# thelondonsmiths/Solex_ser_recon_EN

Measured on AMD Instinct MI355X. Metric: SER frames/sec end-to-end (decode→clahe) + %HBM roofline, 1/2/4/8 MI355X, higher is better.
Workload: dtype u16

## Files before the change

### include/shg_hip.h

```cpp
#ifndef SHG_HIP_H
#define SHG_HIP_H

#include <stddef.h>
#include <stdint.h>

#ifdef __cplusplus
extern "C" {
#endif

#define SHG_ABI_VERSION 16

#define SHG_E_ARG        (-1)
#define SHG_E_WORKSPACE  (-2)
#define SHG_E_UNSUPPORTED (-3)
#define SHG_E_VALUE      (-4)
#define SHG_E_TYPE       (-5)
#define SHG_E_LINALG     (-6)
#define SHG_E_RUNTIME    (-7)
#define SHG_E_QHULL      (-8)
#define SHG_E_ASSERT     (-9)
#define SHG_E_INDEX      (-10)

typedef void* shg_stream_t;

// ... 145 lines not shown
                        int64_t n_cols, int64_t k_offset, int flip_x, shg_stream_t stream);

int shg_extract_columns_minmax(const void* stack, int64_t n_frames, int64_t height, int64_t width,
                               int bytes_per_px, int64_t frame_stride_px, const int32_t* ind_l, const double* lw, const double* rw,
                               int n_shifts, uint16_t* disks, int64_t row_pitch, int64_t plane_stride,
                               int64_t n_cols, int64_t k_offset, int flip_x, uint32_t* minmax_slots, shg_stream_t stream);

int shg_extract_dense_fits(const int32_t* host_shifts, int n_shifts);
int shg_extract_columns_dense(const void* stack, int64_t n_frames, int64_t height, int64_t width, int bytes_per_px,
                              int64_t frame_stride_px, const int32_t* ind_l, const int32_t* base_col, const double* lw,
                              const double* rw, const int32_t* host_shifts, int n_shifts, uint16_t* disks, int64_t row_pitch,
                              int64_t plane_stride, int64_t n_cols, int64_t k_offset, int flip_x, uint32_t* minmax_slots,
                              shg_stream_t stream);

int shg_warp_rows_u16(const uint16_t* src, int64_t h, int64_t w, int64_t src_pitch,
                      double h00, double h01, double h02,
                      uint16_t* dst, int64_t out_h, int64_t out_w, int64_t dst_pitch,
                      uint32_t* minmax, shg_stream_t stream);

int shg_warp_rows_minmax_u16(const uint16_t* src, int64_t h, int64_t w, int64_t src_pitch,
                             double h00, double h01, double h02,
                             uint16_t* dst, int64_t out_h, int64_t out_w, int64_t dst_pitch,
                             const uint32_t* minmax2, shg_stream_t stream);

int shg_warp_rows_wide_fits(const uint16_t* src, int64_t h, int64_t w, int64_t src_pitch,
                            double h00, double h01, double h02,
                            const uint16_t* dst, int64_t out_h, int64_t out_w, int64_t dst_pitch);

#define SHG_TRANSV_MAX_COLS 19456
int shg_rowpair_logratio_stats(const uint16_t* img, int64_t h, int64_t w, int64_t pitch,
                               int64_t y1, int64_t y2, const int32_t* xa, const int32_t* xb,
                               const double* row_factor, double* out, shg_stream_t stream);
int shg_rowpair_logratio_stats_mirrored(const uint16_t* img, int64_t h, int64_t w, int64_t pitch,
                                        int64_t y1, int64_t y2, const int32_t* xa, const int32_t* xb,
                                        const double* row_factor, double* out, double* out_mirror, shg_stream_t stream);

int shg_correlate1d_rows_f64(const double* src, int64_t k, int64_t n, const double* weights, int radius,
                             int symmetric, double* dst, shg_stream_t stream);

int shg_scale_rows_u16(const uint16_t* img, int64_t h, int64_t w, int64_t pitch, const double* c,
                       const double* row_factor, uint16_t* dst, int64_t dst_pitch, shg_stream_t stream);
int shg_scale_rows_vec_fits(const uint16_t* img, int64_t h, int64_t w, int64_t pitch, const uint16_t* dst, int64_t dst_pitch);

int shg_lin_filter_row_sums(const uint16_t* img, int64_t h, int64_t w, int64_t pitch,
                            const double* row_factor, const float* log_lut, const uint8_t* flagged,
                            const int32_t* up, const int32_t* dn, int linlen, double* hl, double* hf,
// ... 269 lines not shown
```

### solex_ser_recon_en_amd/_lib.py

```python
import ctypes
import os
from ctypes import c_double, c_int, c_int32, c_int64, c_size_t, c_uint16, c_uint32, c_void_p

import torch

_HERE = os.path.dirname(os.path.abspath(__file__))
LIB_PATH = os.path.join(_HERE, 'csrc', 'libshg_hip.so')

if not os.path.exists(LIB_PATH):
    raise ImportError(
        'libshg_hip.so is missing (%s). Build it with `python -c "import __graft_entry__ as g; g.build()"` or '
        '`make -C solex_ser_recon_en_amd/csrc`. There is no CPU fallback for the SHG hot path.' % LIB_PATH)

lib = ctypes.CDLL(LIB_PATH)

P = c_void_p
PD = ctypes.POINTER(c_double)
PI64 = ctypes.POINTER(c_int64)


class ScanRequest(ctypes.Structure):
    _fields_ = [('struct_bytes', c_uint32), ('start_phase', c_int32),
                ('stack', P), ('n_frames', c_int64), ('height', c_int64), ('width', c_int64), ('frame_stride_px', c_int64),
                ('bytes_per_px', c_int32), ('flip_x', c_int32),
# ... 73 lines not shown
    'shg_patch_ssd_u16': (c_int, [P, c_int64, P, c_int64, c_int64, c_int64, P, c_int64, c_int, c_int, P, P, P]),
    'shg_stack_combine_field_u16': (c_int, [P, P, P, P, c_int64, c_int64, c_int, c_int, c_int, c_double, c_int, P, c_int64, c_int64, c_int64,
                                            P, c_int64, P]),
    'shg_patch_sharpness_u16': (c_int, [P, c_int64, c_int64, c_int64, P, c_int64, c_int, c_int, P, P, P]),
    'shg_stack_combine_weighted_u16': (c_int, [P, P, P, P, P, c_int64, c_int64, c_int, c_int, c_int, c_double, c_int, P, c_int64, c_int64,
                                               c_int64, P, c_int64, P]),
    'shg_wavelet_workspace_bytes': (c_size_t, [c_int64, c_int64, c_int]),
    'shg_wavelet_sharpen_u16': (c_int, [P, c_int64, c_int64, c_int64, c_int, P, P, P, c_int64, P, P, c_size_t, P]),
    'shg_wavelet_noise_u16': (c_int, [P, c_int64, c_int64, c_int64, P, P, P, c_size_t, P]),
    'shg_rl_workspace_bytes': (c_size_t, [c_int64, c_int64]),
    'shg_rl_deconvolve_u16': (c_int, [P, c_int64, c_int64, c_int64, P, c_int, c_int, P, c_int64, P, P, c_size_t, P]),
    'shg_blur_fits_fused': (c_int, [c_int64, c_int]),
    'shg_blur_row_mean_u16': (c_int, [P, c_int64, c_int64, c_int, c_int, P, P]),
    'shg_blur_argmin_u16': (c_int, [P, c_int64, c_int64, c_int, c_int, c_int64, c_int64, P, P, P]),
    'shg_extract_columns': (c_int, [P, c_int64, c_int64, c_int64, c_int, c_int64, P, P, P, c_int, P, c_int64, c_int64,
                                    c_int64, c_int64, c_int, P]),
    'shg_extract_columns_minmax': (c_int, [P, c_int64, c_int64, c_int64, c_int, c_int64, P, P, P, c_int, P, c_int64, c_int64,
                                           c_int64, c_int64, c_int, P, P]),
    'shg_extract_dense_fits': (c_int, [P, c_int]),
    'shg_extract_columns_dense': (c_int, [P, c_int64, c_int64, c_int64, c_int, c_int64, P, P, P, P, P, c_int, P, c_int64, c_int64, c_int64, c_int64,
                                          c_int, P, P]),
    'shg_warp_rows_minmax_u16': (c_int, [P, c_int64, c_int64, c_int64, c_double, c_double, c_double, P, c_int64, c_int64,
                                         c_int64, P, P]),
    'shg_warp_rows_u16': (c_int, [P, c_int64, c_int64, c_int64, c_double, c_double, c_double, P, c_int64, c_int64,
                                  c_int64, P, P]),
    'shg_warp_rows_wide_fits': (c_int, [P, c_int64, c_int64, c_int64, c_double, c_double, c_double, P, c_int64, c_int64, c_int64]),
    'shg_rowpair_logratio_stats': (c_int, [P, c_int64, c_int64, c_int64, c_int64, c_int64, P, P, P, P, P]),
    'shg_rowpair_logratio_stats_mirrored': (c_int, [P, c_int64, c_int64, c_int64, c_int64, c_int64, P, P, P, P, P, P]),
    'shg_line_order_stats_u16': (c_int, [P, c_int64, c_int64, c_int64, c_int, c_int64, c_int64, P, P, P]),
    'shg_scale_rows_u16': (c_int, [P, c_int64, c_int64, c_int64, P, P, P, c_int64, P]),
    'shg_scale_rows_vec_fits': (c_int, [P, c_int64, c_int64, c_int64, P, c_int64]),
    'shg_correlate1d_rows_f64': (c_int, [P, c_int64, c_int64, P, c_int, c_int, P, P]),
    'shg_lin_filter_row_sums': (c_int, [P, c_int64, c_int64, c_int64, P, P, P, P, P, c_int, P, P, P]),
    'shg_lin_filter_apply': (c_int, [P, c_int64, c_int64, c_int64, P, P, P, c_int, c_int, P, P, P, P, c_int, P, c_int64, P]),
    'shg_crop_pad_u16': (c_int, [P, c_int64, c_int64, c_int64, P, c_int64, c_int64, c_int64, c_int64, c_int64,
                                 c_int, P]),
    'shg_clahe_workspace_bytes': (c_size_t, [c_int, c_int]),
    'shg_clahe_workspace_bytes_for': (c_size_t, [c_int64, c_int64, c_int, c_int]),
    'shg_clahe': (c_int, [P, c_int64, c_int64, c_int64, c_int, c_double, c_int, P, c_int64, P, c_size_t, P]),
    'shg_hist': (c_int, [P, c_int64, c_int64, c_int64, c_int, P, P]),
    'shg_select_u16_workspace_bytes': (c_size_t, [c_int]),
    'shg_select_u16': (c_int, [P, c_int64, c_int64, c_int64, ctypes.POINTER(c_int64), c_int, P, P, c_size_t, P]),
    'shg_rescale_u16': (c_int, [P, c_int64, c_int64, c_int64, c_double, c_double, c_double, P, c_int64, P]),
    'shg_rescale_u8': (c_int, [P, c_int64, c_int64, c_int64, c_double, c_double, c_double, P, c_int64, P]),
    'shg_contrast_stats_workspace_bytes': (c_size_t, [c_int]),
    'shg_contrast_stats_workspace_bytes_for': (c_size_t, [c_int64, c_int64, c_int]),
# ... 224 lines not shown
```

### solex_ser_recon_en_amd/csrc/scan.hip

```cpp
#include <math.h>
#include <string.h>
#include <atomic>
#include <vector>
#include "shg_common.h"

namespace {

constexpr size_t kAlign = 256;
inline size_t up(size_t b) { return (b + kAlign - 1) / kAlign * kAlign; }
inline int64_t round64(int64_t v) { return (v + 63) / 64 * 64; }
inline int64_t floor_div(int64_t a, int64_t b) { int64_t q = a / b; return (a % b != 0 && ((a < 0) != (b < 0))) ? q - 1 : q; }

const double kRadToDeg = 180.0 / 3.141592653589793238462643383279502884;
const double kDegToRad = 3.141592653589793238462643383279502884 / 180.0;

std::atomic<shg_savgol_taps_fn> g_taps_fn{nullptr};

#define SCAN_TRY(expr)                  \
    do {                                \
        if (int e_ = (expr)) return e_; \
    } while (0)

struct Regions {
    size_t mean_ws, extract_ws, limb_ws, mean_pin, extract_pin, limb_pin, process_pin;
// ... 268 lines not shown
    std::vector<double> w_h;
    auto add_warp = [&](int i, uint16_t* dst) {
        const double* hr = i == 0 ? rs->h_first : rs->h_rest;
        w_src.push_back(rq->disks + (size_t)i * rq->disk_plane_stride);
        w_dst.push_back(dst);
        w_mm.push_back(extrema + 2 * i);
        w_h.insert(w_h.end(), hr, hr + 3);
    };
    if (fit_image) add_warp(0, reinterpret_cast<uint16_t*>(arena + rs->fit_image_off));
    std::vector<const uint16_t*> frames((size_t)k);
    std::vector<uint16_t*> det((size_t)k), prod[5];
    for (auto& v : prod) v.resize((size_t)k);
    int64_t j = 0;
    for (int i = 0; i < S; ++i) {
        if (!rq->host_requested[i]) continue;
        uint16_t* f = reinterpret_cast<uint16_t*>(arena + rs->frames_off + (size_t)j * frame_bytes);
        add_warp(i, f);
        frames[j] = f;
        if (detrans) det[j] = reinterpret_cast<uint16_t*>(arena + rs->detrans_off + (size_t)j * frame_bytes);
        for (int p = 0; p < 3; ++p) prod[p][j] = reinterpret_cast<uint16_t*>(arena + rs->products_off + ((size_t)j * 3 + p) * prod_bytes);
        for (int p = 0; p < 2; ++p) prod[3 + p][j] = reinterpret_cast<uint16_t*>(results + ((size_t)j * 2 + p) * prod_bytes);
        ++j;
    }
    if (!w_src.empty())
        SCAN_TRY(shg::warp_rows_batch(w_src.data(), (int64_t)w_src.size(), ih, n_cols, rq->disk_pitch, w_h.data(), w_dst.data(), out_h, out_w, frame_pitch,
                                      w_mm.data(), stream));
    if (k > 0) {
        SCAN_TRY(shg_stage_process_frames(frames.data(), k, out_h, out_w, frame_pitch, rq->transversalium, pl.trans_circle, pl.trans_borders,
                                          pl.taps_ptr, pl.window, rq->host_factors, pl.crop_w, pl.sx0, pl.dx0, pl.ncopy, rq->clip_limit, rq->tiles,
                                          pl.disc[0], pl.disc[1], pl.disc[2], detrans ? det.data() : nullptr, frame_pitch, prod[0].data(),
                                          prod[1].data(), prod[2].data(), prod[3].data(), prod[4].data(), prod_pitch, process_ws, process_ws_bytes,
                                          process_pin, rg.process_pin, stream));
    }
    rs->phase_done = 4;
    return 0;
}
```

### solex_ser_recon_en_amd/csrc/shg_common.h

```cpp
#pragma once
#if defined(__HIPCC__)
#include <hip/hip_runtime.h>
#include <hip/hip_ext.h>
#endif
#include <stdint.h>
#include <stdio.h>
#include <string.h>
#include <type_traits>

#if defined(__HIPCC__)
#define SHG_HD __host__ __device__ __forceinline__
#else
#define SHG_HD inline
#endif

namespace shg {

SHG_HD uint64_t f64_key(double v) {
#if defined(__HIP_DEVICE_COMPILE__)
    const uint64_t b = (uint64_t)__double_as_longlong(v);
#else
    uint64_t b;
    memcpy(&b, &v, sizeof b);
#endif
// ... 111 lines not shown
    template <typename T>
    __device__ __forceinline__ T* at(int i) const { return static_cast<T*>(const_cast<void*>(p[i])); }
};
using PtrBatch = PtrBatchN<kMaxBatch>;
template <int N, typename T>
inline PtrBatchN<N> make_batch_n(T* const* host_ptrs, int first, int count) {
    PtrBatchN<N> b = {};
    for (int i = 0; i < count && i < N; ++i) b.p[i] = host_ptrs[first + i];
    return b;
}
template <typename T>
inline PtrBatch make_batch(T* const* host_ptrs, int first, int count) { return make_batch_n<kMaxBatch>(host_ptrs, first, count); }

int rowpair_stats_batch(const uint16_t* const* host_imgs, int64_t k, int64_t h, int64_t w, int64_t pitch, int64_t y1, int64_t y2,
                        const int32_t* xa, const int32_t* xb, const double* row_factor, double* out, double* out_mirror, shg_stream_t stream);
int scale_rows_batch(const uint16_t* const* host_imgs, int64_t k, int64_t h, int64_t w, int64_t pitch, const double* c,
                     const double* row_factor, uint16_t* const* host_dsts, int64_t dst_pitch, shg_stream_t stream);
int crop_pad_batch(const uint16_t* const* host_srcs, int64_t k, int64_t h, int64_t w, int64_t pitch, uint16_t* const* host_dsts, int64_t nw,
                   int64_t dst_pitch, int64_t sx0, int64_t dx0, int64_t n, int32_t fill, shg_stream_t stream);
int contrast_products_batch(const uint16_t* const* host_frames, int64_t frame_pitch, const uint16_t* const* host_cl1, int64_t cl1_pitch,
                            int64_t k, int64_t h, int64_t w, const double* host_lo_hi6, uint16_t* const* host_hc, uint16_t* const* host_protus,
                            uint16_t* const* host_cc, int64_t dst_pitch, int64_t disc_x0, int64_t disc_y0, int64_t disc_r, shg_stream_t stream,
                            const double* stats5 = nullptr, double g_bright = 0.0, double g_dark = 0.0, double* mirror5 = nullptr);
int warp_rows_batch(const uint16_t* const* host_srcs, int64_t k, int64_t h, int64_t w, int64_t src_pitch, const double* host_h3,
                    uint16_t* const* host_dsts, int64_t out_h, int64_t out_w, int64_t dst_pitch, const uint32_t* const* host_minmax2,
                    shg_stream_t stream);
struct FrameSource {
    const uint16_t* const* host_raw;
    int64_t raw_pitch;
    const double* factors;
    int64_t sx0, dx0, ncopy;
};
bool contrast_stats_batches(int64_t h, int64_t w, int tiles, double clip_limit);
int contrast_stats_batch(const uint16_t* const* host_frames, int64_t k, int64_t h, int64_t w, int64_t pitch, double clip_limit, int tiles,
                         uint16_t* const* host_cl1, int64_t cl1_pitch, const int64_t* ranks_frame2, const int64_t* ranks_cl13, double* out5,
                         void* workspace, size_t workspace_bytes, shg_stream_t stream, const FrameSource* from = nullptr);

constexpr int kWave = 64;
constexpr int kCUs = 256;

__device__ __forceinline__ int lane_id() { return threadIdx.x & (kWave - 1); }

template <typename Op>
__device__ __forceinline__ uint32_t wave_fold_u32(uint32_t v, Op op) {
    v = op(v, (uint32_t)__builtin_amdgcn_update_dpp((int)v, (int)v, 0xB1, 0xf, 0xf, false));
    v = op(v, (uint32_t)__builtin_amdgcn_update_dpp((int)v, (int)v, 0x4E, 0xf, 0xf, false));
    v = op(v, (uint32_t)__builtin_amdgcn_update_dpp((int)v, (int)v, 0x141, 0xf, 0xf, false));
    v = op(v, (uint32_t)__builtin_amdgcn_update_dpp((int)v, (int)v, 0x140, 0xf, 0xf, false));
    const uint32_t r0 = (uint32_t)__builtin_amdgcn_readlane((int)v, 0), r1 = (uint32_t)__builtin_amdgcn_readlane((int)v, 16),
// ... 89 lines not shown
```

### solex_ser_recon_en_amd/csrc/stages.hip

```cpp
#include <math.h>
#include <stdlib.h>
#include <string.h>
#include <algorithm>
#include <vector>
#include "shg_common.h"

namespace {

constexpr size_t kAlign = 256;
inline size_t up(size_t b) { return (b + kAlign - 1) / kAlign * kAlign; }

struct Arena {
    char* base;
    size_t cap, off;
    Arena(void* p, size_t bytes) : base(static_cast<char*>(p)), cap(bytes), off(0) {}
    template <typename T>
    T* take(size_t count) {
        const size_t b = up(count * sizeof(T));
        if (!base || off + b > cap) return nullptr;
        T* p = reinterpret_cast<T*>(base + off);
        off += b;
        return p;
    }
};
// ... 49 lines not shown
    if (n_words == 0) return 0;
    const unsigned blocks = (unsigned)std::min<size_t>((n_words + 255) / 256, 64);
    return shg::launch(k_words, dim3(blocks), dim3(256), 0, st, WordsArgs{static_cast<uint32_t*>(dst), static_cast<const uint32_t*>(src), n_words, nullptr, 0}, "k_words");
}

struct Staging {
    char* host;
    char* dev;
    template <typename T>
    T* on_device(T* host_ptr) const { return reinterpret_cast<T*>(dev + (reinterpret_cast<char*>(host_ptr) - host)); }
};

inline int map_staging(void* host_pinned, Staging* out, const char* who) {
    void* d = nullptr;
    hipError_t e = hipHostGetDevicePointer(&d, host_pinned, 0);
    if (e != hipSuccess || !d) {
        (void)hipGetLastError();
        shg::set_error("%s: host_pinned is not page-locked, GPU-mapped memory (hipHostMalloc / hipHostRegister): %s", who,
                       e != hipSuccess ? hipGetErrorString(e) : "no device address");
        return SHG_E_ARG;
    }
    out->host = static_cast<char*>(host_pinned);
    out->dev = static_cast<char*>(d);
    return 0;
}

inline int64_t slit_rows(int64_t height, int64_t width) { return width > height ? width : height; }
inline int64_t spectral_cols(int64_t height, int64_t width) { return width > height ? height : width; }

}

extern "C" size_t shg_stage_mean_fit_workspace_bytes(int64_t n_frames, int64_t height, int64_t width, int bytes_per_px) {
    if (height <= 0 || width <= 0) return 0;
    const size_t hw = (size_t)height * (size_t)width, ih = (size_t)slit_rows(height, width);
    const size_t acc = n_frames > 0 ? shg_accumulate_workspace_bytes(n_frames, height, width, bytes_per_px) : 0;
    return up(acc) + up(hw * 8) + up(hw * 2) + up(hw * 2) + up(hw * 4) + up(ih * 8) + up(2 * ih * 4) + kAlign;
}

extern "C" size_t shg_stage_mean_fit_host_bytes(int64_t height, int64_t width) {
    if (height <= 0 || width <= 0) return 0;
    const size_t ih = (size_t)slit_rows(height, width);
    return up(ih * 8) + up(2 * ih * 4);
}

extern "C" int shg_stage_mean_fit(const void* stack, int64_t n_frames, int64_t height, int64_t width, int bytes_per_px,
                                  int64_t frame_stride_px, const uint64_t* sum_in, const uint16_t* max_in, int64_t n_total,
// ... 331 lines not shown
        if (host_flags[i]) {
            X[2 * j] = (double)host_points[2 * i] * kFactor;
            X[2 * j + 1] = (double)host_points[2 * i + 1] * kFactor;
            ++j;
        }
    STAGE_TRY(shg_host_limb_geometry(X.data(), n_sel, h, w, host_geom16, host_dims2, kept.data(), &host_counts3[2], host_outline200));
    for (int64_t i = 0, j = 0; i < m; ++i)
        if (host_flags[i]) { if (kept[j]) host_flags[i] |= 2; ++j; }
    return 0;
}

extern "C" size_t shg_stage_process_workspace_bytes(int64_t k, int64_t h, int64_t w, int64_t crop_w, int tiles) {
    if (k <= 0 || h <= 0 || w <= 0) return 0;
    const size_t pitch = ((size_t)std::max(w, crop_w) + 63) / 64 * 64;
    return 2 * up((size_t)h * 4) + 2 * up((size_t)k * h * 8) + up((size_t)k * h * 8) + up(4096 * 8) +
           (size_t)k * up((size_t)h * pitch * 2) + (size_t)k * up(shg_contrast_stats_workspace_bytes_for(h, crop_w > 0 ? crop_w : w, tiles)) + up((size_t)k * 5 * 8) + kAlign;
}

extern "C" size_t shg_stage_process_host_bytes(int64_t k, int64_t h) {
    if (k <= 0 || h <= 0) return 0;
    return 2 * up((size_t)h * 4) + 2 * up((size_t)k * h * 8) + up((size_t)k * h * 8) + up((size_t)k * 5 * 8) + up(4096 * 8);
}

extern "C" int shg_stage_process_frames(const uint16_t* const* host_frames, int64_t k, int64_t h, int64_t w, int64_t pitch,
                                        int transversalium, const double* host_circle3, const double* host_borders4,
                                        const double* host_taps, int64_t window, double* host_factors,
                                        int64_t crop_w, int64_t sx0, int64_t dx0, int64_t ncopy,
                                        double clip_limit, int tiles, int64_t disc_x0, int64_t disc_y0, int64_t disc_r,
                                        uint16_t* const* host_detrans, int64_t detrans_pitch,
                                        uint16_t* const* host_final, uint16_t* const* host_cl1, uint16_t* const* host_hc,
                                        uint16_t* const* host_protus, uint16_t* const* host_cc, int64_t out_pitch,
                                        void* workspace, size_t workspace_bytes, void* host_pinned, size_t host_pinned_bytes,
                                        shg_stream_t stream) {
    SHG_HOST_TIME("stage process_frames");
    SHG_REQUIRE(host_frames && host_final && host_cl1 && host_hc && host_protus && host_cc && workspace && host_pinned, SHG_E_ARG,
                "shg_stage_process_frames: null pointer");
    SHG_REQUIRE(k > 0 && h > 0 && w > 0 && pitch >= w, SHG_E_ARG, "shg_stage_process_frames: bad image size");
    const int64_t out_w = crop_w > 0 ? crop_w : w;
    SHG_REQUIRE(out_pitch >= out_w, SHG_E_ARG, "shg_stage_process_frames: out_pitch < output width");
    hipStream_t st = shg::as_stream(stream);
    Arena dev(workspace, workspace_bytes), pin(host_pinned, host_pinned_bytes);
    int32_t* xa = dev.take<int32_t>((size_t)h);
    int32_t* xb = dev.take<int32_t>((size_t)h);
    double* taps_d = dev.take<double>(4096);
    double* stats = dev.take<double>((size_t)k * h);
    double* interior = dev.take<double>((size_t)k * h);
    double* factors = dev.take<double>((size_t)k * h);
    const size_t tpitch = ((size_t)w + 63) / 64 * 64;
    std::vector<uint16_t*> scaled((size_t)k, nullptr);
    const char* fuse_env = getenv("SHG_FUSE_SCALE");
    const bool fuse_on = !(fuse_env && fuse_env[0] == '0');
    const bool fuse = fuse_on && !host_detrans && shg::contrast_stats_batches(h, crop_w > 0 ? crop_w : w, tiles, clip_limit) && pitch >= w;
    const bool need_tmp = transversalium && crop_w > 0 && !host_detrans && !fuse;
    if (need_tmp)
        for (int64_t i = 0; i < k; ++i) scaled[i] = dev.take<uint16_t>((size_t)h * tpitch);
    const size_t cs_each = up(shg_contrast_stats_workspace_bytes_for(h, out_w, tiles));
    SHG_REQUIRE(cs_each != 0, SHG_E_ARG, "shg_stage_process_frames: unsupported tile count %d", tiles);
    const size_t cs_bytes = (size_t)k * cs_each;
    char* cs_ws = dev.take<char>(cs_bytes);
    double* out5 = dev.take<double>((size_t)k * 5);
    int32_t* h_xa = pin.take<int32_t>((size_t)h);
    int32_t* h_xb = pin.take<int32_t>((size_t)h);
    double* h_taps = pin.take<double>(4096);
    double* h_stats = pin.take<double>((size_t)k * h);
    double* h_interior = pin.take<double>((size_t)k * h);
    double* h_factors = pin.take<double>((size_t)k * h);
    double* h_out5 = pin.take<double>((size_t)k * 5);
    SHG_REQUIRE(xa && xb && stats && interior && factors && taps_d && cs_ws && out5 && (!need_tmp || scaled[k - 1]), SHG_E_WORKSPACE,
                "shg_stage_process_frames: workspace too small");
    SHG_REQUIRE(h_xa && h_xb && h_stats && h_interior && h_factors && h_out5 && h_taps, SHG_E_WORKSPACE, "shg_stage_process_frames: pinned staging area too small");
    Staging stg;
    STAGE_TRY(map_staging(host_pinned, &stg, "shg_stage_process_frames"));

    std::vector<const uint16_t*> cur((size_t)k);
    int64_t cur_pitch = pitch;
    for (int64_t i = 0; i < k; ++i) cur[i] = host_frames[i];
    if (transversalium) {
        SHG_REQUIRE(host_circle3 && host_borders4 && host_taps, SHG_E_ARG, "shg_stage_process_frames: transversalium needs circle, borders, taps");
        const double cx = host_circle3[0], cy = host_circle3[1], r = host_circle3[2];
        const int64_t y1 = (int64_t)ceil(std::max(cy - r, host_borders4[1])), y2 = (int64_t)floor(std::min(cy + r, host_borders4[3]));
        int64_t n = 1;
        bool have_rows = y2 - y1 >= 1;
        const double* use_interior = nullptr;
        if (have_rows) {
            SHG_REQUIRE(y1 >= 0 && y2 <= h, SHG_E_ARG, "shg_stage_process_frames: rows [%lld, %lld) outside the image", (long long)y1, (long long)y2);
            n = y2 - y1;
            STAGE_TRY(shg_host_chord_bounds(cx, cy, r, host_borders4[0], host_borders4[2], y1, y2, w, h_xa, h_xb));
            const bool gpu_interior = window > 3 && window <= n && window / 2 <= 1024 && window <= 4096;
            std::vector<double> rev;
            if (gpu_interior) {
                rev.resize((size_t)window);
                for (int64_t i = 0; i < window; ++i) rev[i] = host_taps[window - 1 - i];
                memcpy(h_taps, rev.data(), (size_t)window * 8);
            }
            const char* plan_end = gpu_interior ? reinterpret_cast<const char*>(h_taps + window) : reinterpret_cast<const char*>(h_xb + n);
            STAGE_TRY(move_words(xa, stg.on_device(h_xa), (size_t)(plan_end - reinterpret_cast<const char*>(h_xa)), st));
            STAGE_TRY(shg::rowpair_stats_batch(host_frames, k, h, w, pitch, y1, y2, xa, xb, nullptr, stats, stg.on_device(h_stats), stream));
            if (gpu_interior) {
                const int radius = (int)(window / 2);
                int sym = 1, anti = 1;
                for (int i = 1; i <= radius; ++i) {
                    if (fabs(rev[radius + i] - rev[radius - i]) > 2.220446049250313e-16) sym = 0;
                    if (fabs(rev[radius + i] + rev[radius - i]) > 2.220446049250313e-16) anti = 0;
                }
                STAGE_TRY(shg_correlate1d_rows_f64(stats, k, n, taps_d, radius, sym ? 1 : (anti ? -1 : 0), stg.on_device(h_interior), stream));
                use_interior = h_interior;
            }
            STAGE_SYNC(st, "shg_stage_process_frames");
        } else {
            for (int64_t i = 0; i < k; ++i) h_stats[i] = 0.0;
        }
        std::vector<double> corr((size_t)k * n);
        STAGE_TRY(shg_host_transversalium_factors(h_stats, use_interior, k, n, host_taps, window, 1, corr.data()));
        for (int64_t i = 0; i < k; ++i) {
            double* c = h_factors + i * h;
            for (int64_t y = 0; y < h; ++y) c[y] = 1.0;
            if (have_rows) memcpy(c + y1, corr.data() + i * n, (size_t)n * 8);
        }
        if (host_factors) memcpy(host_factors, h_factors, (size_t)k * h * 8);
        factors = stg.on_device(h_factors);
      if (!fuse) {
        std::vector<uint16_t*> dsts((size_t)k);
        int64_t dpitch = out_pitch;
        for (int64_t i = 0; i < k; ++i) {
            if (host_detrans) { dsts[i] = host_detrans[i]; dpitch = detrans_pitch; }
            else if (crop_w > 0) { dsts[i] = scaled[i]; dpitch = (int64_t)tpitch; }
            else { dsts[i] = host_final[i]; dpitch = out_pitch; }
            SHG_REQUIRE(dsts[i] && dpitch >= w, SHG_E_ARG, "shg_stage_process_frames: bad de-transversalium output");
// ... 49 lines not shown
```

### solex_ser_recon_en_amd/csrc/warp.hip

```cpp
#include <algorithm>
#include <cmath>
#include "shg_common.h"
#include <type_traits>

namespace {

__global__ void k_minmax_init(uint32_t* mm) {
    mm[0] = 0xffffffffu;
    mm[1] = 0u;
}

__global__ __launch_bounds__(256) void k_minmax(const uint16_t* __restrict__ src, int64_t h, int64_t w, int64_t pitch,
                                                uint32_t* __restrict__ mm) {
    uint32_t lo = 0xffffffffu, hi = 0u;
    for (int64_t y0 = blockIdx.x; y0 < h; y0 += 8 * (int64_t)gridDim.x) {
        for (int64_t x = threadIdx.x; x < w; x += 256) {
            uint32_t v[8];
            bool ok[8];
#pragma unroll
            for (int u = 0; u < 8; ++u) {
                const int64_t y = y0 + u * (int64_t)gridDim.x;
                ok[u] = y < h;
                v[u] = src[(ok[u] ? y : y0) * pitch + x];
            }
// ... 14 lines not shown
    }
    __shared__ uint32_t wlo[4], whi[4];
    if ((threadIdx.x & 63) == 0) { wlo[threadIdx.x >> 6] = lo; whi[threadIdx.x >> 6] = hi; }
    __syncthreads();
    if (threadIdx.x == 0) {
        for (int i = 1; i < 4; ++i) { lo = wlo[i] < lo ? wlo[i] : lo; hi = whi[i] > hi ? whi[i] : hi; }
        atomicMin(&mm[0], lo);
        atomicMax(&mm[1], hi);
    }
}

constexpr int kWarpBatch = 24;
struct WarpRows { double h[kWarpBatch][3]; };

using WarpPtrs = shg::PtrBatchN<kWarpBatch>;
struct WarpArgs {
    WarpPtrs srcs;
    int64_t h, w, pitch;
    WarpRows rows;
    WarpPtrs dsts;
    int64_t out_h, out_w, dst_pitch;
    WarpPtrs mms;
    uint32_t nv_magic, nv_shift;
};

template <int WARP_ROWS>
__global__ __launch_bounds__(256) void k_warp_rows(const WarpArgs kargs) {
    const WarpPtrs& srcs = kargs.srcs;
    const WarpPtrs& dsts = kargs.dsts;
    const WarpPtrs& mms = kargs.mms;
    const int64_t h = kargs.h, w = kargs.w, pitch = kargs.pitch, out_h = kargs.out_h, out_w = kargs.out_w, dst_pitch = kargs.dst_pitch;
    const WarpRows& rows = kargs.rows;
    const uint16_t* __restrict__ src = srcs.at<const uint16_t>(blockIdx.z);
    uint16_t* __restrict__ dst = dsts.at<uint16_t>(blockIdx.z);
    const uint32_t* __restrict__ mm = mms.at<const uint32_t>(blockIdx.z);
    const double h00 = rows.h[blockIdx.z][0], h01 = rows.h[blockIdx.z][1], h02 = rows.h[blockIdx.z][2];
    const int c = (int)(blockIdx.x * 256 + threadIdx.x);
    const int ra = (int)blockIdx.y * WARP_ROWS;
    if (c >= out_w) return;
    double dc[WARP_ROWS];
    uint32_t v0[WARP_ROWS], v1[WARP_ROWS];
    bool in0[WARP_ROWS], in1[WARP_ROWS];
    const bool sane = fabs(h00) < 1e300 && fabs(h01) < 1e300 && fabs(h02) < 1e300;
    const uint32_t wu = (uint32_t)w;
    const double xc = h00 * (double)c;
#pragma unroll
    for (int rr = 0; rr < WARP_ROWS; ++rr) {
        const int r = ra + rr;
        const double x = xc + h01 * (double)r + h02;
        const double x0 = floor(x);
// ... 6 lines not shown
        const uint16_t* row = src + (int64_t)(row_ok ? r : 0) * pitch;
        v0[rr] = row[in0[rr] ? i0 : 0];
        v1[rr] = row[in1[rr] ? i1 : 0];
    }
    const uint32_t cval = src[0];
    const double lo = (double)mm[0], hi = (double)mm[1];
#pragma unroll
    for (int rr = 0; rr < WARP_ROWS; ++rr) {
        const int r = ra + rr;
        if (r >= out_h) break;
        const double left = (double)(in0[rr] ? v0[rr] : cval), right = (double)(in1[rr] ? v1[rr] : cval);
        double v = (1.0 - dc[rr]) * left + dc[rr] * right;
        v = fmin(fmax(v, lo), hi);
        dst[(int64_t)r * dst_pitch + c] = (uint16_t)(int)v;
    }
}

typedef unsigned int __attribute__((ext_vector_type(4))) u32x4_t;
typedef unsigned int __attribute__((ext_vector_type(3))) u32x3_t;
constexpr int kWarpPairs = 22;
template <int ITER>
__global__ __launch_bounds__(256) __attribute__((amdgpu_waves_per_eu(7))) void k_warp_rows8(const WarpArgs kargs) {
    __shared__ uint32_t win[4][kWarpPairs][64];
    const int64_t h = kargs.h, w = kargs.w, pitch = kargs.pitch, out_h = kargs.out_h, out_w = kargs.out_w, dst_pitch = kargs.dst_pitch;
    const uint16_t* __restrict__ src = kargs.srcs.at<const uint16_t>(blockIdx.z);
    uint16_t* __restrict__ dst = kargs.dsts.at<uint16_t>(blockIdx.z);
    const uint32_t* __restrict__ mm = kargs.mms.at<const uint32_t>(blockIdx.z);
    const double h00 = kargs.rows.h[blockIdx.z][0], h01 = kargs.rows.h[blockIdx.z][1], h02 = kargs.rows.h[blockIdx.z][2];
    const uint32_t nv = (uint32_t)((out_w + 7) / 8), total = nv * (uint32_t)out_h;
    const int lane = threadIdx.x & 63, wave = threadIdx.x >> 6;
    uint32_t (*const my)[64] = win[wave];
    const uint32_t cval = src[0];
    const int lo_i = (int)mm[0], hi_i = (int)mm[1];
    const double k00 = h00 * 0x1p+52;
    const uint32_t wu = (uint32_t)w;
    const int w_last = (int)w - 1, last_piece = (int)pitch - 8;

    auto place = [&](int it, int& r, int& c, int& ws, double& hr, double& x) {
        const uint32_t flat = ((uint32_t)blockIdx.x * ITER + (uint32_t)it) * 256u + threadIdx.x;
        const uint32_t f = flat < total ? flat : total - 1;
        r = (int)(__umulhi(f, kargs.nv_magic) >> kargs.nv_shift);
        c = (int)(f - (uint32_t)r * nv) * 8;
        hr = h01 * (double)r;
        x = h00 * (double)c + hr + h02;
        const int i0 = __double2int_rz(floor(x));
        ws = min(max(i0, 0), w_last) & ~7;
// ... 100 lines not shown
                                 uint32_t* minmax, shg_stream_t stream) {
    SHG_REQUIRE(src && dst && minmax, SHG_E_ARG, "shg_warp_rows_u16: null pointer");
    SHG_REQUIRE(h > 0 && w > 0 && out_h > 0 && out_w > 0, SHG_E_ARG, "shg_warp_rows_u16: empty image");
    SHG_REQUIRE(src_pitch >= w && dst_pitch >= out_w, SHG_E_ARG, "shg_warp_rows_u16: pitch smaller than width");
    SHG_REQUIRE(out_h < 65536, SHG_E_UNSUPPORTED, "shg_warp_rows_u16: more than 65535 rows");
    hipStream_t st = shg::as_stream(stream);
    { SHG_PROF("minmax", st); k_minmax_init<<<1, 1, 0, st>>>(minmax); }
    int64_t blocks = h < 256 ? h : 256;
    { SHG_PROF("minmax", st); k_minmax<<<(unsigned)blocks, 256, 0, st>>>(src, h, w, src_pitch, minmax); }
    if (int e = shg::check_launch("k_minmax")) return e;
    const double h3[3] = {h00, h01, h02};
    const uint32_t* mm = minmax;
    return shg::warp_rows_batch(&src, 1, h, w, src_pitch, h3, &dst, out_h, out_w, dst_pitch, &mm, stream);
}

extern "C" int shg_warp_rows_minmax_u16(const uint16_t* src, int64_t h, int64_t w, int64_t src_pitch, double h00, double h01,
                                        double h02, uint16_t* dst, int64_t out_h, int64_t out_w, int64_t dst_pitch,
                                        const uint32_t* minmax2, shg_stream_t stream) {
    SHG_REQUIRE(src && dst && minmax2, SHG_E_ARG, "shg_warp_rows_minmax_u16: null pointer");
    const double h3[3] = {h00, h01, h02};
    return shg::warp_rows_batch(&src, 1, h, w, src_pitch, h3, &dst, out_h, out_w, dst_pitch, &minmax2, stream);
}

int shg::warp_rows_batch(const uint16_t* const* host_srcs, int64_t k, int64_t h, int64_t w, int64_t src_pitch, const double* host_h3,
                         uint16_t* const* host_dsts, int64_t out_h, int64_t out_w, int64_t dst_pitch, const uint32_t* const* host_minmax2,
                         shg_stream_t stream) {
    SHG_REQUIRE(host_srcs && host_h3 && host_dsts && host_minmax2 && k > 0, SHG_E_ARG, "shg_warp_rows_minmax_u16: null pointer");
    SHG_REQUIRE(h > 0 && w > 0 && out_h > 0 && out_w > 0, SHG_E_ARG, "shg_warp_rows_minmax_u16: empty image");
    SHG_REQUIRE(src_pitch >= w && dst_pitch >= out_w, SHG_E_ARG, "shg_warp_rows_minmax_u16: pitch smaller than width");
    SHG_REQUIRE(out_h < 65536 && out_w < (1ll << 30) && w < (1ll << 30) && h < (1ll << 30), SHG_E_UNSUPPORTED, "shg_warp_rows_minmax_u16: image too large");
    for (int64_t i = 0; i < k; ++i) SHG_REQUIRE(host_srcs[i] && host_dsts[i] && host_minmax2[i], SHG_E_ARG, "shg_warp_rows_minmax_u16: null image");
    hipStream_t st = shg::as_stream(stream);
    SHG_PROF("warp", st);
    for (int64_t i0 = 0; i0 < k; i0 += kWarpBatch) {
        const int m = (int)std::min<int64_t>(kWarpBatch, k - i0);
        WarpRows rows = {};
        for (int d = 0; d < m; ++d)
            for (int j = 0; j < 3; ++j) rows.h[d][j] = host_h3[3 * (i0 + d) + j];
        const uint64_t nv = (uint64_t)((out_w + 7) / 8);
        uint32_t nv_shift = 0;
        while ((2ull << nv_shift) < nv) ++nv_shift;
        const uint32_t nv_magic = nv >= 2 ? (uint32_t)(((1ull << (32 + nv_shift)) + nv - 1) / nv) : 0u;
        const WarpArgs args{shg::make_batch_n<kWarpBatch>(host_srcs, (int)i0, m), h, w, src_pitch, rows, shg::make_batch_n<kWarpBatch>(host_dsts, (int)i0, m),
                            out_h, out_w, dst_pitch, shg::make_batch_n<kWarpBatch>(host_minmax2, (int)i0, m), nv_magic, nv_shift};
        const bool wide_ok = [] { const char* e = getenv("SHG_WARP_WIDE"); return !e || atoi(e) != 0; }();
        bool wide = wide_ok;
        for (int d = 0; d < m && wide; ++d)
            wide = shg_warp_rows_wide_fits(host_srcs[i0 + d], h, w, src_pitch, rows.h[d][0], rows.h[d][1], rows.h[d][2], host_dsts[i0 + d], out_h, out_w, dst_pitch) != 0;
        if (wide) {
            const int64_t vecs = out_h * ((out_w + 7) / 8);
            const bool few = vecs * m < 4 * 256 * 2048;
            auto go8 = [&](auto I) {
                dim3 grid((unsigned)((vecs + 256 * I.value - 1) / (256 * I.value)), 1u, (unsigned)m);
                return shg::launch(k_warp_rows8<I.value>, grid, dim3(256), 0, st, args, "k_warp_rows8");
            };
            if (int e = few ? go8(std::integral_constant<int, 1>{}) : go8(std::integral_constant<int, 4>{})) return e;
            continue;
        }
        const int64_t gx = (out_w + 255) / 256;
        int rows_per_lane = gx * ((out_h + 7) / 8) * m >= kWarpWideAbove ? 8 : 4;
        if (warp_rows_forced()) rows_per_lane = warp_rows_forced();
        auto go = [&](auto R) {
            dim3 grid((unsigned)gx, (unsigned)((out_h + R.value - 1) / R.value), (unsigned)m);
            return shg::launch(k_warp_rows<R.value>, grid, dim3(256), 0, st, args, "k_warp_rows");
        };
        const int e = rows_per_lane == 16 ? go(std::integral_constant<int, 16>{})
                    : rows_per_lane == 8 ? go(std::integral_constant<int, 8>{}) : go(std::integral_constant<int, 4>{});
// ... 5 lines not shown
```

Measured before the change: 6.099 million.

## Carry transversalium plan upload inside warp kernel to skip separate copy

The host-side transversalium plan (chord bounds, reversed taps, symmetry) is now computed before the warp launch. The warp kernels copy the plan words from mapped pinned memory to the device workspace using their first 64 workgroups. The process stage reuses that staged plan through a thread-local pointer and skips its own move_words launch. This removes one small copy launch per call, at the cost of a hidden thread-local handoff and extra work in the first warp blocks.

Result: no change. 6.060 million (-0.6%).

```diff
diff --git a/include/shg_hip.h b/include/shg_hip.h
--- a/include/shg_hip.h
+++ b/include/shg_hip.h
@@ -191,6 +191,12 @@
                              double h00, double h01, double h02,
                              uint16_t* dst, int64_t out_h, int64_t out_w, int64_t dst_pitch,
                              const uint32_t* minmax2, shg_stream_t stream);
+
+int shg_warp_rows_side_copy_u16(const uint16_t* src, int64_t h, int64_t w, int64_t src_pitch,
+                                double h00, double h01, double h02,
+                                uint16_t* dst, int64_t out_h, int64_t out_w, int64_t dst_pitch,
+                                const uint32_t* minmax2, uint32_t* side_dst, const uint32_t* side_src, size_t n_words,
+                                shg_stream_t stream);
 
 int shg_warp_rows_wide_fits(const uint16_t* src, int64_t h, int64_t w, int64_t src_pitch,
                             double h00, double h01, double h02,
diff --git a/solex_ser_recon_en_amd/_lib.py b/solex_ser_recon_en_amd/_lib.py
--- a/solex_ser_recon_en_amd/_lib.py
+++ b/solex_ser_recon_en_amd/_lib.py
@@ -119,6 +119,8 @@
                                           c_int, P, P]),
     'shg_warp_rows_minmax_u16': (c_int, [P, c_int64, c_int64, c_int64, c_double, c_double, c_double, P, c_int64, c_int64,
                                          c_int64, P, P]),
+    'shg_warp_rows_side_copy_u16': (c_int, [P, c_int64, c_int64, c_int64, c_double, c_double, c_double, P, c_int64, c_int64,
+                                            c_int64, P, P, P, c_size_t, P]),
     'shg_warp_rows_u16': (c_int, [P, c_int64, c_int64, c_int64, c_double, c_double, c_double, P, c_int64, c_int64,
                                   c_int64, P, P]),
     'shg_warp_rows_wide_fits': (c_int, [P, c_int64, c_int64, c_int64, c_double, c_double, c_double, P, c_int64, c_int64, c_int64]),
diff --git a/solex_ser_recon_en_amd/csrc/scan.hip b/solex_ser_recon_en_amd/csrc/scan.hip
--- a/solex_ser_recon_en_amd/csrc/scan.hip
+++ b/solex_ser_recon_en_amd/csrc/scan.hip
@@ -314,10 +314,16 @@
         for (int p = 0; p < 2; ++p) prod[3 + p][j] = reinterpret_cast<uint16_t*>(results + ((size_t)j * 2 + p) * prod_bytes);
         ++j;
     }
+    shg::ProcessPlanWords plan_words;
+    const bool carry = k > 0 && rq->transversalium;
+    if (carry)
+        SCAN_TRY(shg::process_plan_words(out_h, out_w, pl.trans_circle, pl.trans_borders, pl.taps_ptr, pl.window, process_ws, process_ws_bytes, process_pin,
+                                         rg.process_pin, &plan_words));
     if (!w_src.empty())
         SCAN_TRY(shg::warp_rows_batch(w_src.data(), (int64_t)w_src.size(), ih, n_cols, rq->disk_pitch, w_h.data(), w_dst.data(), out_h, out_w, frame_pitch,
-                                      w_mm.data(), stream));
+                                      w_mm.data(), stream, carry ? &plan_words.copy : nullptr));
     if (k > 0) {
+        if (carry) shg::t_process_plan_staged = &plan_words;
         SCAN_TRY(shg_stage_process_frames(frames.data(), k, out_h, out_w, frame_pitch, rq->transversalium, pl.trans_circle, pl.trans_borders,
                                           pl.taps_ptr, pl.window, rq->host_factors, pl.crop_w, pl.sx0, pl.dx0, pl.ncopy, rq->clip_limit, rq->tiles,
                                           pl.disc[0], pl.disc[1], pl.disc[2], detrans ? det.data() : nullptr, frame_pitch, prod[0].data(),
diff --git a/solex_ser_recon_en_amd/csrc/shg_common.h b/solex_ser_recon_en_amd/csrc/shg_common.h
--- a/solex_ser_recon_en_amd/csrc/shg_common.h
+++ b/solex_ser_recon_en_amd/csrc/shg_common.h
@@ -157,9 +157,23 @@
                             int64_t k, int64_t h, int64_t w, const double* host_lo_hi6, uint16_t* const* host_hc, uint16_t* const* host_protus,
                             uint16_t* const* host_cc, int64_t dst_pitch, int64_t disc_x0, int64_t disc_y0, int64_t disc_r, shg_stream_t stream,
                             const double* stats5 = nullptr, double g_bright = 0.0, double g_dark = 0.0, double* mirror5 = nullptr);
+struct SideCopy {
+    uint32_t* dst;
+    const uint32_t* src;
+    size_t n_words;
+};
 int warp_rows_batch(const uint16_t* const* host_srcs, int64_t k, int64_t h, int64_t w, int64_t src_pitch, const double* host_h3,
                     uint16_t* const* host_dsts, int64_t out_h, int64_t out_w, int64_t dst_pitch, const uint32_t* const* host_minmax2,
-                    shg_stream_t stream);
+                    shg_stream_t stream, const SideCopy* side = nullptr);
+struct ProcessPlanWords {
+    int64_t y1, y2;
+    bool have_rows, gpu_interior;
+    int symmetry;
+    SideCopy copy;
+};
+int process_plan_words(int64_t h, int64_t w, const double* host_circle3, const double* host_borders4, const double* host_taps, int64_t window,
+                       void* workspace, size_t workspace_bytes, void* host_pinned, size_t host_pinned_bytes, ProcessPlanWords* out);
+extern thread_local const ProcessPlanWords* t_process_plan_staged;
 struct FrameSource {
     const uint16_t* const* host_raw;
     int64_t raw_pitch;
diff --git a/solex_ser_recon_en_amd/csrc/stages.hip b/solex_ser_recon_en_amd/csrc/stages.hip
--- a/solex_ser_recon_en_amd/csrc/stages.hip
+++ b/solex_ser_recon_en_amd/csrc/stages.hip
@@ -95,6 +95,35 @@
     }
     out->host = static_cast<char*>(host_pinned);
     out->dev = static_cast<char*>(d);
+    return 0;
+}
+
+int plan_words(int64_t h, int64_t w, const double* host_circle3, const double* host_borders4, const double* host_taps, int64_t window,
+               int32_t* xa, int32_t* h_xa, int32_t* h_xb, double* h_taps, const Staging& stg, shg::ProcessPlanWords* out) {
+    SHG_REQUIRE(host_circle3 && host_borders4 && host_taps, SHG_E_ARG, "shg_stage_process_frames: transversalium needs circle, borders, taps");
+    const double cx = host_circle3[0], cy = host_circle3[1], r = host_circle3[2];
+    *out = shg::ProcessPlanWords{};
+    out->y1 = (int64_t)ceil(std::max(cy - r, host_borders4[1]));
+    out->y2 = (int64_t)floor(std::min(cy + r, host_borders4[3]));
+    out->have_rows = out->y2 - out->y1 >= 1;
+    if (!out->have_rows) return 0;
+    const int64_t y1 = out->y1, y2 = out->y2, n = y2 - y1;
+    SHG_REQUIRE(y1 >= 0 && y2 <= h, SHG_E_ARG, "shg_stage_process_frames: rows [%lld, %lld) outside the image", (long long)y1, (long long)y2);
+    STAGE_TRY(shg_host_chord_bounds(cx, cy, r, host_borders4[0], host_borders4[2], y1, y2, w, h_xa, h_xb));
+    out->gpu_interior = window > 3 && window <= n && window / 2 <= 1024 && window <= 4096;
+    if (out->gpu_interior) {
+        for (int64_t i = 0; i < window; ++i) h_taps[i] = host_taps[window - 1 - i];
+        const int64_t radius = window / 2;
+        int sym = 1, anti = 1;
+        for (int64_t i = 1; i <= radius; ++i) {
+            if (fabs(h_taps[radius + i] - h_taps[radius - i]) > 2.220446049250313e-16) sym = 0;
+            if (fabs(h_taps[radius + i] + h_taps[radius - i]) > 2.220446049250313e-16) anti = 0;
+        }
+        out->symmetry = sym ? 1 : (anti ? -1 : 0);
+    }
+    const char* plan_end = out->gpu_interior ? reinterpret_cast<const char*>(h_taps + window) : reinterpret_cast<const char*>(h_xb + n);
+    const size_t bytes = (size_t)(plan_end - reinterpret_cast<const char*>(h_xa));
+    out->copy = shg::SideCopy{reinterpret_cast<uint32_t*>(xa), reinterpret_cast<const uint32_t*>(stg.on_device(h_xa)), (bytes + 3) / 4};
     return 0;
 }
 
@@ -472,6 +501,25 @@
     return 2 * up((size_t)h * 4) + 2 * up((size_t)k * h * 8) + up((size_t)k * h * 8) + up((size_t)k * 5 * 8) + up(4096 * 8);
 }
 
+thread_local const shg::ProcessPlanWords* shg::t_process_plan_staged = nullptr;
+
+int shg::process_plan_words(int64_t h, int64_t w, const double* host_circle3, const double* host_borders4, const double* host_taps, int64_t window,
+                            void* workspace, size_t workspace_bytes, void* host_pinned, size_t host_pinned_bytes, shg::ProcessPlanWords* out) {
+    SHG_REQUIRE(out && workspace && host_pinned && h > 0 && w > 0, SHG_E_ARG, "shg_stage_process_frames: null pointer");
+    *out = shg::ProcessPlanWords{};
+    Arena dev(workspace, workspace_bytes), pin(host_pinned, host_pinned_bytes);
+    int32_t* xa = dev.take<int32_t>((size_t)h);
+    int32_t* xb = dev.take<int32_t>((size_t)h);
+    double* taps_d = dev.take<double>(4096);
+    int32_t* h_xa = pin.take<int32_t>((size_t)h);
+    int32_t* h_xb = pin.take<int32_t>((size_t)h);
+    double* h_taps = pin.take<double>(4096);
+    if (!xa || !xb || !taps_d || !h_xa || !h_xb || !h_taps) return 0;
+    Staging stg;
+    STAGE_TRY(map_staging(host_pinned, &stg, "shg_stage_process_frames"));
+    return plan_words(h, w, host_circle3, host_borders4, host_taps, window, xa, h_xa, h_xb, h_taps, stg, out);
+}
+
 extern "C" int shg_stage_process_frames(const uint16_t* const* host_frames, int64_t k, int64_t h, int64_t w, int64_t pitch,
                                         int transversalium, const double* host_circle3, const double* host_borders4,
                                         const double* host_taps, int64_t window, double* host_factors,
@@ -483,6 +531,8 @@
                                         void* workspace, size_t workspace_bytes, void* host_pinned, size_t host_pinned_bytes,
                                         shg_stream_t stream) {
     SHG_HOST_TIME("stage process_frames");
+    const shg::ProcessPlanWords* staged = shg::t_process_plan_staged;
+    shg::t_process_plan_staged = nullptr;
     SHG_REQUIRE(host_frames && host_final && host_cl1 && host_hc && host_protus && host_cc && workspace && host_pinned, SHG_E_ARG,
                 "shg_stage_process_frames: null pointer");
     SHG_REQUIRE(k > 0 && h > 0 && w > 0 && pitch >= w, SHG_E_ARG, "shg_stage_process_frames: bad image size");
@@ -526,34 +576,23 @@
     int64_t cur_pitch = pitch;
     for (int64_t i = 0; i < k; ++i) cur[i] = host_frames[i];
     if (transversalium) {
-        SHG_REQUIRE(host_circle3 && host_borders4 && host_taps, SHG_E_ARG, "shg_stage_process_frames: transversalium needs circle, borders, taps");
-        const double cx = host_circle3[0], cy = host_circle3[1], r = host_circle3[2];
-        const int64_t y1 = (int64_t)ceil(std::max(cy - r, host_borders4[1])), y2 = (int64_t)floor(std::min(cy + r, host_borders4[3]));
+        shg::ProcessPlanWords own;
+        const bool carried = staged && staged->copy.n_words > 0 && staged->copy.dst == reinterpret_cast<uint32_t*>(xa) &&
+                             staged->copy.src == reinterpret_cast<const uint32_t*>(stg.on_device(h_xa));
+        if (!carried) {
+            STAGE_TRY(plan_words(h, w, host_circle3, host_borders4, host_taps, window, xa, h_xa, h_xb, h_taps, stg, &own));
+            staged = &own;
+        }
+        const int64_t y1 = staged->y1, y2 = staged->y2;
         int64_t n = 1;
-        bool have_rows = y2 - y1 >= 1;
+        const bool have_rows = staged->have_rows;
         const double* use_interior = nullptr;
         if (have_rows) {
-            SHG_REQUIRE(y1 >= 0 && y2 <= h, SHG_E_ARG, "shg_stage_process_frames: rows [%lld, %lld) outside the image", (long long)y1, (long long)y2);
             n = y2 - y1;
-            STAGE_TRY(shg_host_chord_bounds(cx, cy, r, host_borders4[0], host_borders4[2], y1, y2, w, h_xa, h_xb));
-            const bool gpu_interior = window > 3 && window <= n && window / 2 <= 1024 && window <= 4096;
-            std::vector<double> rev;
-            if (gpu_interior) {
-                rev.resize((size_t)window);
-                for (int64_t i = 0; i < window; ++i) rev[i] = host_taps[window - 1 - i];
-                memcpy(h_taps, rev.data(), (size_t)window * 8);
-            }
-            const char* plan_end = gpu_interior ? reinterpret_cast<const char*>(h_taps + window) : reinterpret_cast<const char*>(h_xb + n);
-            STAGE_TRY(move_words(xa, stg.on_device(h_xa), (size_t)(plan_end - reinterpret_cast<const char*>(h_xa)), st));
+            if (!carried) STAGE_TRY(move_words(staged->copy.dst, staged->copy.src, staged->copy.n_words * 4, st));
             STAGE_TRY(shg::rowpair_stats_batch(host_frames, k, h, w, pitch, y1, y2, xa, xb, nullptr, stats, stg.on_device(h_stats), stream));
-            if (gpu_interior) {
-                const int radius = (int)(window / 2);
-                int sym = 1, anti = 1;
-                for (int i = 1; i <= radius; ++i) {
-                    if (fabs(rev[radius + i] - rev[radius - i]) > 2.220446049250313e-16) sym = 0;
-                    if (fabs(rev[radius + i] + rev[radius - i]) > 2.220446049250313e-16) anti = 0;
-                }
-                STAGE_TRY(shg_correlate1d_rows_f64(stats, k, n, taps_d, radius, sym ? 1 : (anti ? -1 : 0), stg.on_device(h_interior), stream));
+            if (staged->gpu_interior) {
+                STAGE_TRY(shg_correlate1d_rows_f64(stats, k, n, taps_d, (int)(window / 2), staged->symmetry, stg.on_device(h_interior), stream));
                 use_interior = h_interior;
             }
             STAGE_SYNC(st, "shg_stage_process_frames");
diff --git a/solex_ser_recon_en_amd/csrc/warp.hip b/solex_ser_recon_en_amd/csrc/warp.hip
--- a/solex_ser_recon_en_amd/csrc/warp.hip
+++ b/solex_ser_recon_en_amd/csrc/warp.hip
@@ -60,10 +60,24 @@
     int64_t out_h, out_w, dst_pitch;
     WarpPtrs mms;
     uint32_t nv_magic, nv_shift;
+    uint32_t* side_dst;
+    const uint32_t* side_src;
+    size_t side_words;
 };
+
+constexpr uint32_t kWarpSideGroups = 64;
+__device__ __forceinline__ void warp_side_copy(const WarpArgs& kargs) {
+    const uint64_t wg = blockIdx.x + (uint64_t)gridDim.x * (blockIdx.y + (uint64_t)gridDim.y * blockIdx.z);
+    if (wg >= kWarpSideGroups) return;
+    const uint64_t all = (uint64_t)gridDim.x * gridDim.y * gridDim.z, groups = all < kWarpSideGroups ? all : kWarpSideGroups;
+    uint32_t* __restrict__ dst = kargs.side_dst;
+    const uint32_t* __restrict__ src = kargs.side_src;
+    for (size_t i = (size_t)wg * 256 + threadIdx.x; i < kargs.side_words; i += (size_t)groups * 256) dst[i] = src[i];
+}
 
 template <int WARP_ROWS>
 __global__ __launch_bounds__(256) void k_warp_rows(const WarpArgs kargs) {
+    if (kargs.side_words) warp_side_copy(kargs);
     const WarpPtrs& srcs = kargs.srcs;
     const WarpPtrs& dsts = kargs.dsts;
     const WarpPtrs& mms = kargs.mms;
@@ -116,6 +130,7 @@
 template <int ITER>
 __global__ __launch_bounds__(256) __attribute__((amdgpu_waves_per_eu(7))) void k_warp_rows8(const WarpArgs kargs) {
     __shared__ uint32_t win[4][kWarpPairs][64];
+    if (kargs.side_words) warp_side_copy(kargs);
     const int64_t h = kargs.h, w = kargs.w, pitch = kargs.pitch, out_h = kargs.out_h, out_w = kargs.out_w, dst_pitch = kargs.dst_pitch;
     const uint16_t* __restrict__ src = kargs.srcs.at<const uint16_t>(blockIdx.z);
     uint16_t* __restrict__ dst = kargs.dsts.at<uint16_t>(blockIdx.z);
@@ -262,10 +277,23 @@
     return shg::warp_rows_batch(&src, 1, h, w, src_pitch, h3, &dst, out_h, out_w, dst_pitch, &minmax2, stream);
 }
 
+extern "C" int shg_warp_rows_side_copy_u16(const uint16_t* src, int64_t h, int64_t w, int64_t src_pitch, double h00, double h01,
+                                           double h02, uint16_t* dst, int64_t out_h, int64_t out_w, int64_t dst_pitch,
+                                           const uint32_t* minmax2, uint32_t* side_dst, const uint32_t* side_src, size_t n_words,
+                                           shg_stream_t stream) {
+    SHG_REQUIRE(src && dst && minmax2, SHG_E_ARG, "shg_warp_rows_side_copy_u16: null pointer");
+    const double h3[3] = {h00, h01, h02};
+    const shg::SideCopy side{side_dst, side_src, n_words};
+    return shg::warp_rows_batch(&src, 1, h, w, src_pitch, h3, &dst, out_h, out_w, dst_pitch, &minmax2, stream, &side);
+}
+
 int shg::warp_rows_batch(const uint16_t* const* host_srcs, int64_t k, int64_t h, int64_t w, int64_t src_pitch, const double* host_h3,
                          uint16_t* const* host_dsts, int64_t out_h, int64_t out_w, int64_t dst_pitch, const uint32_t* const* host_minmax2,
-                         shg_stream_t stream) {
+                         shg_stream_t stream, const shg::SideCopy* side) {
     SHG_REQUIRE(host_srcs && host_h3 && host_dsts && host_minmax2 && k > 0, SHG_E_ARG, "shg_warp_rows_minmax_u16: null pointer");
+    SHG_REQUIRE(!side || side->n_words == 0 || (side->dst && side->src), SHG_E_ARG, "shg_warp_rows_minmax_u16: side copy without its pointers");
+    SHG_REQUIRE(!side || ((reinterpret_cast<uintptr_t>(side->dst) | reinterpret_cast<uintptr_t>(side->src)) & 3) == 0, SHG_E_ARG,
+                "shg_warp_rows_minmax_u16: side copy not 4-byte aligned");
     SHG_REQUIRE(h > 0 && w > 0 && out_h > 0 && out_w > 0, SHG_E_ARG, "shg_warp_rows_minmax_u16: empty image");
     SHG_REQUIRE(src_pitch >= w && dst_pitch >= out_w, SHG_E_ARG, "shg_warp_rows_minmax_u16: pitch smaller than width");
     SHG_REQUIRE(out_h < 65536 && out_w < (1ll << 30) && w < (1ll << 30) && h < (1ll << 30), SHG_E_UNSUPPORTED, "shg_warp_rows_minmax_u16: image too large");
@@ -281,8 +309,10 @@
         uint32_t nv_shift = 0;
         while ((2ull << nv_shift) < nv) ++nv_shift;
         const uint32_t nv_magic = nv >= 2 ? (uint32_t)(((1ull << (32 + nv_shift)) + nv - 1) / nv) : 0u;
+        const bool carry = side && side->n_words > 0 && i0 == 0;
         const WarpArgs args{shg::make_batch_n<kWarpBatch>(host_srcs, (int)i0, m), h, w, src_pitch, rows, shg::make_batch_n<kWarpBatch>(host_dsts, (int)i0, m),
-                            out_h, out_w, dst_pitch, shg::make_batch_n<kWarpBatch>(host_minmax2, (int)i0, m), nv_magic, nv_shift};
+                            out_h, out_w, dst_pitch, shg::make_batch_n<kWarpBatch>(host_minmax2, (int)i0, m), nv_magic, nv_shift,
+                            carry ? side->dst : nullptr, carry ? side->src : nullptr, carry ? side->n_words : 0};
         const bool wide_ok = [] { const char* e = getenv("SHG_WARP_WIDE"); return !e || atoi(e) != 0; }();
         bool wide = wide_ok;
         for (int d = 0; d < m && wide; ++d)
```
